# SamuelCancilla2/radar-point-cloud-tracking

Hardware: NVIDIA B200
Metric: fused_frames_per_s_through_stdbscan (higher is better)
Workload: dtype f32 (points) / f64 (neighbour test) / i32 (labels)

## Files before the change

### radar_point_cloud_tracking_b200/csrc/spoke.cu

```cuda
#include <stdlib.h>

#include "common.cuh"

namespace {

constexpr int SK_THREADS = 256;
constexpr int SK_WARPS = SK_THREADS / 32;
constexpr int SK_TILE = 4096;
constexpr int SK_WORDS = SK_TILE / 32;
constexpr int SK_BATCH = 8;
constexpr int SK_BATCH_CELLS = SK_BATCH * 128;
constexpr int SK_BATCHES = SK_TILE / SK_BATCH_CELLS;
constexpr int SK_GROUP = 4;
constexpr int SK_ENTRIES = SK_GROUP * 32;
constexpr int SK_CTAS_PER_SM = 4;

struct FastDiv { uint32_t mul, shift, d; };
inline FastDiv make_fastdiv(uint32_t d) {
    FastDiv f; f.d = d; f.mul = 0; f.shift = 0;
    if (d <= 1) return f;
    uint32_t l = 0;
    while ((1ull << l) < d) ++l;
    f.mul = (uint32_t)((((1ull << l) - d) << 32) / d + 1);
    f.shift = l;
    return f;
}
__device__ __forceinline__ uint32_t fastdiv(uint32_t n, const FastDiv& f) {
    if (f.d <= 1) return n;
    uint32_t t = __umulhi(f.mul, n);
    return (t + ((n - t) >> 1)) >> (f.shift - 1);
}

struct SpokeGeom {
    int64_t total_tiles;
    int sweep_cells;
    int tiles_per_sweep;
    int n_bins;
    int n_spokes;
};

__device__ __forceinline__ unsigned set_gt(float a, float b) {
    unsigned r;
    asm("set.gt.u32.f32 %0, %1, %2;" : "=r"(r) : "f"(a), "f"(b));
    return r;
}

struct LaneBits { unsigned b0, b1, b2, b3; };
__device__ __forceinline__ LaneBits lane_bits(unsigned lane) {
    const unsigned sh = 4u * (lane & 7u);
    return LaneBits{1u << sh, 2u << sh, 4u << sh, 8u << sh};
}
__device__ __forceinline__ unsigned nibble(const float4& v, float thr, const LaneBits& lb) {
    return (set_gt(v.x, thr) & lb.b0) | (set_gt(v.y, thr) & lb.b1) | (set_gt(v.z, thr) & lb.b2) | (set_gt(v.w, thr) & lb.b3);
}

struct ThrArg {
    float thr;
    unsigned lb4;
    int none;
};
inline ThrArg make_thr(float thr) {
    ThrArg a; a.thr = thr; a.lb4 = 0; a.none = 0;
    if (!(thr == thr)) { a.none = 1; return a; }
    if (thr < 0.f) return a;
    const double lb = floor((double)thr) + 1.0;
    if (lb > 255.0) { a.none = 1; return a; }
    a.lb4 = (unsigned)lb * 0x01010101u;
    return a;
}
template <typename T> struct Elem;
template <> struct Elem<float>   { static constexpr int ALIGN_CELLS = 4;  static constexpr int WARPS = 8; };
template <> struct Elem<uint8_t> { static constexpr int ALIGN_CELLS = 16; static constexpr int WARPS = 16; };

__device__ __forceinline__ unsigned u8_bits4(unsigned word, const ThrArg& t) {
    const unsigned r = t.none ? 0u : __vcmpgeu4(word, t.lb4);
    return ((r & 0x01010101u) * 0x01020408u) >> 24;
}
__device__ __forceinline__ unsigned nibble_u8(unsigned word, const ThrArg& t, unsigned sh) {
    const unsigned r = t.none ? 0u : __vcmpgeu4(word, t.lb4);
    return (((r & 0x01010101u) * 0x01020408u) >> 24) << sh;
}
template <typename T>
__device__ __forceinline__ unsigned batch_nibble(const unsigned char* __restrict__ batch, int k, unsigned lane, const ThrArg& t,
                                                 const LaneBits& lb) {
    if (sizeof(T) == 4) return nibble(reinterpret_cast<const float4*>(batch)[k * 32 + lane], t.thr, lb);
    return nibble_u8(reinterpret_cast<const unsigned*>(batch)[k * 32 + lane], t, 4u * (lane & 7u));
}

__device__ __forceinline__ unsigned butterfly8(const unsigned (&nib)[8], unsigned lane) {
    unsigned a4[4], a2[2];
#pragma unroll
    for (int i = 0; i < 4; ++i) {
        const bool hi = lane & 1u;
        unsigned keep = hi ? nib[2 * i + 1] : nib[2 * i];
        unsigned give = hi ? nib[2 * i] : nib[2 * i + 1];
        a4[i] = keep | __shfl_xor_sync(0xffffffffu, give, 1);
    }
#pragma unroll
    for (int i = 0; i < 2; ++i) {
        const bool hi = lane & 2u;
        unsigned keep = hi ? a4[2 * i + 1] : a4[2 * i];
        unsigned give = hi ? a4[2 * i] : a4[2 * i + 1];
        a2[i] = keep | __shfl_xor_sync(0xffffffffu, give, 2);
    }
    const bool hi = lane & 4u;
    unsigned keep = hi ? a2[1] : a2[0];
    unsigned give = hi ? a2[0] : a2[1];
    return keep | __shfl_xor_sync(0xffffffffu, give, 4);
}

template <typename T>
struct TileRef { const T* src; int valid; };
template <typename T>
__device__ __forceinline__ TileRef<T> tile_ref(const T* echo, const SpokeGeom& g, long long tile) {
    const int w = (int)(tile / g.tiles_per_sweep);
    const int cell0 = (int)(tile - (long long)w * g.tiles_per_sweep) * SK_TILE;
    return TileRef<T>{echo + (int64_t)w * g.sweep_cells + cell0, min(SK_TILE, g.sweep_cells - cell0)};
}

template <typename T> constexpr int mt_threads() { return Elem<T>::WARPS * 32 + 32; }

template <int TILES>
struct MtMeta {
    long long first_tile;
    int n_tiles;
    int valid[TILES];
    unsigned cnt[TILES];
};
template <int TILES, int STAGE_BYTES, int STAGES>
struct __align__(128) MtSmem {
    unsigned char ring[STAGES][STAGE_BYTES];
    unsigned long long full[STAGES];
    unsigned long long empty[STAGES];
    MtMeta<TILES> meta[STAGES];
};
template <typename T, int STAGE_BYTES> __host__ __device__ constexpr int mt_tiles() { return STAGE_BYTES / (SK_TILE * (int)sizeof(T)); }
template <int STAGE_BYTES> __host__ __device__ constexpr int mt_chunk_stages() {
    return (256 * 1024) / STAGE_BYTES > 0 ? (256 * 1024) / STAGE_BYTES : 1;
}
template <typename T, int STAGE_BYTES, int STAGES> constexpr int mt_smem_bytes() {
    return (int)sizeof(MtSmem<mt_tiles<T, STAGE_BYTES>(), STAGE_BYTES, STAGES>) + 128;
}

__device__ __forceinline__ uint32_t smem_u32(const void* p) { return (uint32_t)__cvta_generic_to_shared(p); }
__device__ __forceinline__ void mbar_init(unsigned long long* bar, uint32_t count) {
    asm volatile("mbarrier.init.shared::cta.b64 [%0], %1;" ::"r"(smem_u32(bar)), "r"(count) : "memory");
}
__device__ __forceinline__ void mbar_arrive(unsigned long long* bar) {
    asm volatile("mbarrier.arrive.shared::cta.b64 _, [%0];" ::"r"(smem_u32(bar)) : "memory");
}
__device__ __forceinline__ void mbar_expect_tx(unsigned long long* bar, uint32_t bytes) {
    asm volatile("mbarrier.arrive.expect_tx.shared::cta.b64 _, [%0], %1;" ::"r"(smem_u32(bar)), "r"(bytes) : "memory");
}
__device__ __forceinline__ void mbar_wait(unsigned long long* bar, uint32_t parity) {
    asm volatile(
        "{\n"
        ".reg .pred p;\n"
        "MT_WAIT:\n"
        "mbarrier.try_wait.parity.shared::cta.b64 p, [%0], %1;\n"
        "@p bra.uni MT_DONE;\n"
        "bra.uni MT_WAIT;\n"
        "MT_DONE:\n"
        "}\n" ::"r"(smem_u32(bar)), "r"(parity) : "memory");
}
__device__ __forceinline__ void bulk_g2s(void* dst, const void* src, uint32_t bytes, unsigned long long* bar, unsigned long long policy) {
    if (policy)
        asm volatile("cp.async.bulk.shared::cluster.global.mbarrier::complete_tx::bytes.L2::cache_hint [%0], [%1], %2, [%3], %4;"
                     ::"r"(smem_u32(dst)), "l"(src), "r"(bytes), "r"(smem_u32(bar)), "l"(policy) : "memory");
    else
        asm volatile("cp.async.bulk.shared::cluster.global.mbarrier::complete_tx::bytes [%0], [%1], %2, [%3];"
                     ::"r"(smem_u32(dst)), "l"(src), "r"(bytes), "r"(smem_u32(bar)) : "memory");
}
__device__ __forceinline__ unsigned long long l2_evict_first_policy() {
    unsigned long long p;
    asm volatile("createpolicy.fractional.L2::evict_first.b64 %0, 1.0;" : "=l"(p));
    return p;
}

template <typename T, int MT_STAGE_BYTES, int MT_STAGES>
__global__ void __launch_bounds__(mt_threads<T>(), 1)
spoke_mask_tma_kernel(const T* __restrict__ echo, const SpokeGeom g, const ThrArg threshold,
                      uint32_t* __restrict__ mask, uint32_t* __restrict__ tile_count, unsigned* __restrict__ ticket, const int l2_hint) {
    constexpr int MT_TILES = mt_tiles<T, MT_STAGE_BYTES>();
    constexpr int MT_WARPS = Elem<T>::WARPS;
    constexpr int MT_STAGE_BATCHES = MT_TILES * SK_BATCHES;
    constexpr int MT_CHUNK = mt_chunk_stages<MT_STAGE_BYTES>();
    static_assert(MT_TILES >= 1 && MT_TILES * SK_TILE * sizeof(T) == MT_STAGE_BYTES, "a stage is a whole number of tiles");
    using Smem = MtSmem<MT_TILES, MT_STAGE_BYTES, MT_STAGES>;
    extern __shared__ __align__(128) unsigned char smem_raw[];
    Smem& sm = *reinterpret_cast<Smem*>((reinterpret_cast<uintptr_t>(smem_raw) + 127) & ~uintptr_t(127));
    const unsigned lane = rb_lane();
    const int warp = threadIdx.x >> 5;
    if (threadIdx.x == 0) {
#pragma unroll
        for (int i = 0; i < MT_STAGES; ++i) {
            mbar_init(&sm.full[i], 1);
            mbar_init(&sm.empty[i], MT_WARPS);
#pragma unroll
            for (int t = 0; t < MT_TILES; ++t) sm.meta[i].cnt[t] = 0;
        }
        asm volatile("fence.mbarrier_init.release.cluster;" ::: "memory");
        asm volatile("fence.proxy.async.shared::cta;" ::: "memory");
    }
    __syncthreads();
    const long long n_stages = (g.total_tiles + MT_TILES - 1) / MT_TILES;

    if (warp == MT_WARPS) {
        static_assert(MT_TILES <= 32, "one lane per tile");
        auto flush = [&](int s) {
            MtMeta<MT_TILES>& m = sm.meta[s];
            if ((int)lane < m.n_tiles) {
                tile_count[m.first_tile + lane] = m.cnt[lane];
                m.cnt[lane] = 0;
            }
            __syncwarp();
        };
        const unsigned long long policy = l2_hint ? l2_evict_first_policy() : 0ull;
        long long chunk = blockIdx.x;
        int it = 0;
        auto recycle = [&](int s) {
            if (it >= MT_STAGES) {
                mbar_wait(&sm.empty[s], (uint32_t)(it / MT_STAGES - 1) & 1u);
                flush(s);
            }
        };
        while (true) {
            unsigned tk = 0;
            if (lane == 0) tk = atomicAdd(ticket, 1u);
            const long long st0 = chunk * MT_CHUNK;
            if (st0 >= n_stages) {
                const int s = it % MT_STAGES;
                recycle(s);
                if (lane == 0) {
                    sm.meta[s].first_tile = -1;
                    sm.meta[s].n_tiles = 0;
                    mbar_arrive(&sm.full[s]);
                }
                break;
            }
            const long long st1 = min(st0 + (long long)MT_CHUNK, n_stages);
            long long my_tile = st0 * MT_TILES + lane;
            int my_w = (int)(my_tile / g.tiles_per_sweep);
            int my_tis = (int)(my_tile - (long long)my_w * g.tiles_per_sweep);
            for (long long st = st0; st < st1; ++st) {
                const int s = it % MT_STAGES;
                recycle(s);
                MtMeta<MT_TILES>& m = sm.meta[s];
                const long long t0 = st * MT_TILES;
                const int nt = (int)min((long long)MT_TILES, g.total_tiles - t0);
                int v = 0;
                const T* src = nullptr;
                if ((int)lane < nt) {
                    const int cell0 = my_tis * SK_TILE;
                    v = min(SK_TILE, g.sweep_cells - cell0);
                    src = echo + (int64_t)my_w * g.sweep_cells + cell0;
                }
                my_tile += MT_TILES;
                my_tis += MT_TILES;
                while (my_tis >= g.tiles_per_sweep) { my_tis -= g.tiles_per_sweep; ++my_w; }
                if ((int)lane < MT_TILES) m.valid[lane] = v;
                if (lane == 0) { m.first_tile = t0; m.n_tiles = nt; }
                const uint32_t bytes = __reduce_add_sync(0xffffffffu, (uint32_t)v * (uint32_t)sizeof(T));
                const bool all_full = __all_sync(0xffffffffu, (int)lane >= nt || v == SK_TILE);
                if (lane == 0) mbar_expect_tx(&sm.full[s], bytes);
                __syncwarp();
                if (all_full) {
                    if (lane == 0) bulk_g2s(&sm.ring[s][0], src, bytes, &sm.full[s], policy);
                } else if (v > 0) {
                    bulk_g2s(&sm.ring[s][(size_t)lane * SK_TILE * sizeof(T)], src, (uint32_t)v * (uint32_t)sizeof(T), &sm.full[s], policy);
                }
                ++it;
            }
            chunk = (long long)gridDim.x + (long long)__shfl_sync(0xffffffffu, tk, 0);
        }
        for (int j = max(0, it - (MT_STAGES - 1)); j < it; ++j) {
            const int s = j % MT_STAGES;
            mbar_wait(&sm.empty[s], (uint32_t)(j / MT_STAGES) & 1u);
            flush(s);
        }
        return;
    }

    const LaneBits lb = lane_bits(lane);
    const unsigned word_slot = (lane & 7u) * 4u + (lane >> 3);
    for (int it = 0;; ++it) {
        const int s = it % MT_STAGES;
        mbar_wait(&sm.full[s], (uint32_t)(it / MT_STAGES) & 1u);
        MtMeta<MT_TILES>& m = sm.meta[s];
        const long long t0 = m.first_tile;
        if (t0 < 0) break;
        const int nt = m.n_tiles;
#pragma unroll
        for (int b = warp; b < MT_STAGE_BATCHES; b += MT_WARPS) {
            const int t = b / SK_BATCHES;
            if (t >= nt) break;
            const int valid = m.valid[t] - (b % SK_BATCHES) * SK_BATCH_CELLS;
            const unsigned char* __restrict__ batch = sm.ring[s] + (size_t)b * SK_BATCH_CELLS * sizeof(T);
            uint32_t* __restrict__ mw = mask + (t0 + t) * SK_WORDS + (b % SK_BATCHES) * 32;
            unsigned word;
            if (sizeof(T) == 1 && valid >= SK_BATCH_CELLS) {
                const uint4* __restrict__ q = reinterpret_cast<const uint4*>(batch);
                const uint4 h0 = q[lane], h1 = q[32 + lane];
                unsigned b0 = u8_bits4(h0.x, threshold) | (u8_bits4(h0.y, threshold) << 4) | (u8_bits4(h0.z, threshold) << 8) |
                              (u8_bits4(h0.w, threshold) << 12);
                unsigned b1 = u8_bits4(h1.x, threshold) | (u8_bits4(h1.y, threshold) << 4) | (u8_bits4(h1.z, threshold) << 8) |
                              (u8_bits4(h1.w, threshold) << 12);
                const unsigned sh16 = (lane & 1u) * 16u;
                b0 <<= sh16; b1 <<= sh16;
                b0 |= __shfl_xor_sync(0xffffffffu, b0, 1);
                b1 |= __shfl_xor_sync(0xffffffffu, b1, 1);
                word = (lane & 1u) ? b1 : b0;
                mw[(lane & 1u) * 16u + (lane >> 1)] = word;
            } else {
                unsigned nib[SK_BATCH];
                if (valid >= SK_BATCH_CELLS) {
#pragma unroll
                    for (int k = 0; k < SK_BATCH; ++k) nib[k] = batch_nibble<T>(batch, k, lane, threshold, lb);
                } else {
#pragma unroll
                    for (int k = 0; k < SK_BATCH; ++k) {
                        const int c = k * 128 + (int)lane * 4;
                        nib[k] = c < valid ? batch_nibble<T>(batch, k, lane, threshold, lb) : 0u;
                    }
                }
                word = butterfly8(nib, lane);
                mw[word_slot] = word;
            }
            const unsigned c = __reduce_add_sync(0xffffffffu, __popc(word));
            if (lane == 0 && c) atomicAdd(&m.cnt[t], c);
        }
        __syncwarp();
        if (lane == 0) mbar_arrive(&sm.empty[s]);
    }
}

template <typename T, bool VEC>
__global__ void __launch_bounds__(SK_THREADS, SK_CTAS_PER_SM)
spoke_mask_kernel(const T* __restrict__ echo, const SpokeGeom g, const float threshold,
                  uint32_t* __restrict__ mask, uint32_t* __restrict__ tile_count) {
    static_assert(!VEC || sizeof(T) == 4, "128-bit path is float32 only");
    const unsigned lane = rb_lane();
    const LaneBits lb = lane_bits(lane);
    const unsigned sh = 4u * (lane & 7u);
    const unsigned word_slot = (lane & 7u) * 4u + (lane >> 3);
    const long long n_warps = (long long)gridDim.x * SK_WARPS;
    for (long long tile = (long long)blockIdx.x * SK_WARPS + (threadIdx.x >> 5); tile < g.total_tiles; tile += n_warps) {
        const TileRef<T> tr = tile_ref<T>(echo, g, tile);
        const int valid = tr.valid;
        const T* __restrict__ src = tr.src;
        uint32_t* __restrict__ mw = mask + tile * SK_WORDS;
        unsigned cnt = 0;
#pragma unroll 1
        for (int b = 0; b < SK_BATCHES; ++b) {
            const int c0 = b * SK_BATCH_CELLS + (int)lane * 4;
            unsigned nib[SK_BATCH];
            if (VEC) {
                const float* __restrict__ fsrc = reinterpret_cast<const float*>(src);
                if (valid == SK_TILE) {
                    float4 v[SK_BATCH];
#pragma unroll
                    for (int k = 0; k < SK_BATCH; ++k) v[k] = rb_ld_stream4(fsrc + c0 + k * 128);
#pragma unroll
                    for (int k = 0; k < SK_BATCH; ++k) nib[k] = nibble(v[k], threshold, lb);
                } else {
#pragma unroll
                    for (int k = 0; k < SK_BATCH; ++k) {
                        const int c = c0 + k * 128;
                        nib[k] = c < valid ? nibble(rb_ld_stream4(fsrc + c), threshold, lb) : 0u;
                    }
                }
            } else {
#pragma unroll
                for (int k = 0; k < SK_BATCH; ++k) {
                    const int c = c0 + k * 128;
                    unsigned m = 0;
#pragma unroll
                    for (int i = 0; i < 4; ++i)
                        if (c + i < valid) m |= (unsigned)((float)__ldg(src + c + i) > threshold) << i;
                    nib[k] = m << sh;
                }
            }
            const unsigned word = butterfly8(nib, lane);
            cnt += __popc(word);
            mw[b * 32 + word_slot] = word;
        }
        cnt = __reduce_add_sync(0xffffffffu, cnt);
        if (lane == 0) tile_count[tile] = cnt;
    }
}

constexpr int SO_THREADS = 512;

template <typename T>
__device__ __forceinline__ T block_exclusive_scan(T v, T* s_warp, T* total) {
    const unsigned lane = rb_lane(), warp = threadIdx.x >> 5;
    T incl = v;
#pragma unroll
    for (int d = 1; d < 32; d <<= 1) {
        T o = __shfl_up_sync(0xffffffffu, incl, d);
        if ((int)lane >= d) incl += o;
    }
    if (lane == 31) s_warp[warp] = incl;
    __syncthreads();
    T before = 0, all = 0;
#pragma unroll
    for (int i = 0; i < SO_THREADS / 32; ++i) {
        T c = s_warp[i];
        if (i < (int)warp) before += c;
        all += c;
    }
    __syncthreads();
    *total = all;
    return before + incl - v;
}

__global__ void __launch_bounds__(SO_THREADS)
spoke_offsets_kernel(const uint32_t* __restrict__ tile_count, uint32_t* __restrict__ tile_prefix, int tiles_per_sweep,
                     int64_t n_sweeps, int stride, uint32_t* __restrict__ sweep_total, int64_t* __restrict__ sweep_base,
                     unsigned* __restrict__ done, unsigned* __restrict__ ticket) {
    __shared__ uint32_t s_warp[SO_THREADS / 32];
    __shared__ unsigned long long s_warp64[SO_THREADS / 32];
    __shared__ bool s_last;
    const int64_t w = blockIdx.x;
    const uint32_t* __restrict__ cnt = tile_count + w * tiles_per_sweep;
    uint32_t* __restrict__ pfx = tile_prefix + w * tiles_per_sweep;
    uint32_t carry = 0;
    for (int t0 = 0; t0 < tiles_per_sweep; t0 += SO_THREADS) {
        const int t = t0 + (int)threadIdx.x;
        uint32_t v = t < tiles_per_sweep ? cnt[t] : 0u, total;
        uint32_t e = block_exclusive_scan<uint32_t>(v, s_warp, &total);
        if (t < tiles_per_sweep) pfx[t] = carry + e;
        carry += total;
    }
    if (threadIdx.x == 0) {
        sweep_total[w] = carry;
        __threadfence();
        s_last = atomicAdd(done, 1u) == (unsigned)gridDim.x - 1u;
    }
    __syncthreads();
    if (!s_last) return;
    __threadfence();
    unsigned long long base = 0;
    for (int64_t w0 = 0; w0 < n_sweeps; w0 += SO_THREADS) {
        const int64_t ww = w0 + threadIdx.x;
        const unsigned long long m = ww < n_sweeps ? *(volatile uint32_t*)(sweep_total + ww) : 0u;
        unsigned long long kept = (m + (unsigned)stride - 1u) / (unsigned)stride, total;
        unsigned long long e = block_exclusive_scan<unsigned long long>(kept, s_warp64, &total);
        if (ww < n_sweeps) sweep_base[ww] = (int64_t)(base + e);
        base += total;
    }
    if (threadIdx.x == 0) {
        sweep_base[n_sweeps] = (int64_t)base;
        *done = 0;
        *ticket = 0;
    }
}

template <typename T>
struct EmitArgs {
    const T* echo;
    const float* cos_tab;
    const float* sin_tab;
    const float* range_res;
    const float* ranges;
    const int32_t* sweep_gain;
    const uint32_t* mask;
    const uint32_t* tile_count;
    const uint32_t* tile_prefix;
    const int64_t* sweep_base;
    float* x;
    float* y;
    float* inten;
    int32_t* gain;
    int64_t cap;
    int64_t total_groups;
    int groups_per_sweep;
    SpokeGeom g;
    int stride;
    FastDiv div_stride, div_bins;
};

__device__ __forceinline__ int select_bit(uint32_t word, uint32_t o) {
    int pos = 0;
    uint32_t c;
    c = __popc(word & 0xffffu); if (o >= c) { o -= c; pos += 16; word >>= 16; }
    c = __popc(word & 0xffu);   if (o >= c) { o -= c; pos += 8;  word >>= 8; }
    c = __popc(word & 0xfu);    if (o >= c) { o -= c; pos += 4;  word >>= 4; }
    c = __popc(word & 0x3u);    if (o >= c) { o -= c; pos += 2;  word >>= 2; }
    c = word & 1u;              if (o >= c) { pos += 1; }
    return pos;
}

template <typename T>
__global__ void __launch_bounds__(SK_THREADS) spoke_emit_kernel(const EmitArgs<T> a) {
    __shared__ uint4 s_mask[SK_WARPS][SK_ENTRIES];
    __shared__ uint32_t s_rank[SK_WARPS][SK_ENTRIES];
    const unsigned lane = rb_lane();
    const int warp = threadIdx.x >> 5;
    const int64_t gidx = (int64_t)blockIdx.x * SK_WARPS + warp;
    if (gidx >= a.total_groups) return;
    const int w = (int)(gidx / a.groups_per_sweep);
    const int tile0 = (int)(gidx - (int64_t)w * a.groups_per_sweep) * SK_GROUP;
    const int ntile = min(SK_GROUP, a.g.tiles_per_sweep - tile0);
    const int64_t tile_base = (int64_t)w * a.g.tiles_per_sweep + tile0;

    uint32_t my_cnt = 0, my_pfx = 0;
    if ((int)lane < ntile) { my_cnt = a.tile_count[tile_base + lane]; my_pfx = a.tile_prefix[tile_base + lane]; }
    const uint32_t r_begin = __shfl_sync(0xffffffffu, my_pfx, 0);
    const uint32_t r_end = __shfl_sync(0xffffffffu, my_pfx + my_cnt, ntile - 1);
    const uint32_t s = (uint32_t)a.stride;
    const uint32_t q0 = fastdiv(r_begin + s - 1u, a.div_stride), q1 = fastdiv(r_end + s - 1u, a.div_stride);
    if (q0 >= q1) return;

    const uint4* __restrict__ mask4 = reinterpret_cast<const uint4*>(a.mask) + tile_base * 32;
    uint4 m[SK_GROUP];
#pragma unroll
    for (int t = 0; t < SK_GROUP; ++t) {
        const uint32_t c = __shfl_sync(0xffffffffu, my_cnt, t);
        m[t] = (t < ntile && c) ? mask4[t * 32 + lane] : make_uint4(0u, 0u, 0u, 0u);
    }
#pragma unroll
    for (int t = 0; t < SK_GROUP; ++t) {
        const uint32_t c = __popc(m[t].x) + __popc(m[t].y) + __popc(m[t].z) + __popc(m[t].w);
        uint32_t incl = c;
#pragma unroll
        for (int d = 1; d < 32; d <<= 1) {
            uint32_t o = __shfl_up_sync(0xffffffffu, incl, d);
            if ((int)lane >= d) incl += o;
        }
        const uint32_t pfx = __shfl_sync(0xffffffffu, my_pfx, t);
        s_mask[warp][t * 32 + lane] = m[t];
        s_rank[warp][t * 32 + lane] = t < ntile ? pfx + incl - c : 0xffffffffu;
    }
    __syncwarp();

    const long long out_base = a.sweep_base[w];
    const int gain_label = a.sweep_gain[w];
    const int64_t tab_off = (int64_t)w * a.g.n_spokes;
    const int64_t cell_off = (int64_t)w * a.g.sweep_cells;
    const uint32_t* __restrict__ rk = s_rank[warp];
    for (uint32_t q = q0 + lane; q < q1; q += 32) {
        const uint32_t r = q * s;
        int e = 0;
#pragma unroll
        for (int step = SK_ENTRIES / 2; step >= 1; step >>= 1)
            if (rk[e + step] <= r) e += step;
        uint32_t o = r - rk[e];
        const uint4 mm = s_mask[warp][e];
        uint32_t word = mm.x;
        int wi = 0;
        uint32_t c = __popc(mm.x);
        if (o >= c) { o -= c; word = mm.y; wi = 1; c = __popc(mm.y);
            if (o >= c) { o -= c; word = mm.z; wi = 2; c = __popc(mm.z);
                if (o >= c) { o -= c; word = mm.w; wi = 3; } } }
        const int cell = (tile0 + (e >> 5)) * SK_TILE + (e & 31) * 128 + wi * 32 + select_bit(word, o);
        const long long pos = out_base + q;
        if (pos < a.cap) {
            const int sp = (int)fastdiv((uint32_t)cell, a.div_bins);
            const int j = cell - sp * a.g.n_bins;
            const float val = (float)__ldg(a.echo + cell_off + cell);
            const float cs = __ldg(a.cos_tab + tab_off + sp), sn = __ldg(a.sin_tab + tab_off + sp);
            const float rng = a.ranges ? __ldg(a.ranges + cell_off + cell)
                                       : __fmul_rn(__ldg(a.range_res + tab_off + sp), (float)j);
            a.x[pos] = __fmul_rn(rng, cs);
            a.y[pos] = __fmul_rn(rng, sn);
            a.inten[pos] = val;
            a.gain[pos] = gain_label;
        }
    }
}

__global__ void frame_offsets_kernel(const int64_t* __restrict__ sweep_base, int64_t n_frames, int gpf,
                                     int64_t* __restrict__ frame_off) {
    int64_t f = (int64_t)blockIdx.x * blockDim.x + threadIdx.x;
    if (f <= n_frames) frame_off[f] = sweep_base[f * gpf];
}

__global__ void expand_times_kernel(const int64_t* __restrict__ frame_off, const float* __restrict__ frame_ids,
                                    int64_t n_frames, float* __restrict__ times) {
    for (int64_t f = blockIdx.x; f < n_frames; f += gridDim.x) {
        int64_t b = frame_off[f], e = frame_off[f + 1];
        float id = frame_ids[f];
        for (int64_t i = b + threadIdx.x; i < e; i += blockDim.x) times[i] = id;
    }
}

__global__ void polar_grid_kernel(const float* __restrict__ ranges, const float* __restrict__ cs,
                                  const float* __restrict__ sn, int64_t total, int m, float* __restrict__ x,
                                  float* __restrict__ y) {
    for (int64_t i = (int64_t)blockIdx.x * blockDim.x + threadIdx.x; i < total; i += (int64_t)gridDim.x * blockDim.x) {
        int64_t r = i / m;
        float rg = ranges[i];
        x[i] = __fmul_rn(rg, cs[r]);
        y[i] = __fmul_rn(rg, sn[r]);
    }
}

}

extern "C" int rb_polar_to_cartesian(rb_ctx* ctx, const float* ranges, const float* cos_tab, const float* sin_tab,
                                     int64_t n_rows, int n_cols, float* x, float* y, void* stream_) {
    RB_REQUIRE(ctx, "ctx is NULL");
    RB_REQUIRE(n_rows >= 0 && n_cols >= 0, "negative size");
    int64_t total = n_rows * n_cols;
    if (total == 0) return RB_OK;
    RB_REQUIRE(ranges && cos_tab && sin_tab && x && y, "NULL argument");
    cudaStream_t stream = (cudaStream_t)stream_;
    int blocks = (int)(rb_div_up(total, 256 * 4) < (int64_t)ctx->sm_count * 16 ? rb_div_up(total, 256 * 4)
                                                                               : (int64_t)ctx->sm_count * 16);
    RB_CUDA(rb_launch(ctx, polar_grid_kernel, dim3(blocks), dim3(256), 0, stream, ranges, cos_tab, sin_tab, total, n_cols, x, y));
    RB_LAUNCH_CHECK(ctx);
    return RB_OK;
}

template <typename T, int STAGE_BYTES, int STAGES>
int launch_mask_tma(rb_ctx* ctx, const T* echo, const SpokeGeom& g, const ThrArg& thr, uint32_t* mask, uint32_t* tile_count,
                    unsigned* ticket, cudaStream_t stream) {
    constexpr int smem = mt_smem_bytes<T, STAGE_BYTES, STAGES>();
    constexpr int ring_id = STAGE_BYTES == 64 * 1024 ? 0 : STAGE_BYTES == 48 * 1024 ? 3 : (STAGES == 4 ? 1 : 2);
    const unsigned bit = 1u << (ring_id * 2 + (sizeof(T) == 1 ? 1 : 0));
    auto kernel = spoke_mask_tma_kernel<T, STAGE_BYTES, STAGES>;
    if (!(ctx->attr_spoke_mask & bit)) {
        RB_CUDA(cudaFuncSetAttribute(kernel, cudaFuncAttributeMaxDynamicSharedMemorySize, smem));
        ctx->attr_spoke_mask |= bit;
    }
    const int64_t want_blocks = rb_div_up(g.total_tiles, (int64_t)mt_tiles<T, STAGE_BYTES>() * mt_chunk_stages<STAGE_BYTES>());
    const unsigned blocks = (unsigned)(want_blocks < ctx->sm_count ? want_blocks : ctx->sm_count);
    RB_CUDA(rb_launch_prio(ctx, true, kernel, dim3(blocks), dim3(mt_threads<T>()), (size_t)smem, stream, echo, g, thr, mask, tile_count, ticket,
                      ctx->opt_spoke_l2_hint));
    return RB_OK;
}

#include <mutex>
static std::mutex g_gate_mu;
static cudaEvent_t g_gate_ev[64];

struct MaskGate {
    rb_ctx* ctx;
    cudaStream_t stream;
    bool held = false;
    int enter() {
        if (!ctx->opt_mask_gate || ctx->device < 0 || ctx->device >= 64) return RB_OK;
        g_gate_mu.lock();
        held = true;
        cudaEvent_t& ev = g_gate_ev[ctx->device];
        if (!ev) RB_CUDA(cudaEventCreateWithFlags(&ev, cudaEventDisableTiming));
        else RB_CUDA(cudaStreamWaitEvent(stream, ev, 0));
        return RB_OK;
    }
    void leave() {
        if (!held) return;
        held = false;
        cudaEventRecord(g_gate_ev[ctx->device], stream);
        g_gate_mu.unlock();
    }
    ~MaskGate() { leave(); }
};

template <typename T>
int spoke_to_points_impl(rb_ctx* ctx, const T* echo, const float* cos_tab, const float* sin_tab,
                         const float* range_res, const float* ranges, const int32_t* sweep_gain, int64_t n_sweeps,
                         int n_spokes, int n_bins, float threshold, int stride, float* x, float* y,
                         float* inten, int32_t* gain, int64_t cap, int64_t* sweep_base, void* stream_) {
    RB_REQUIRE(ctx, "ctx is NULL");
    RB_REQUIRE(n_sweeps >= 0 && n_spokes >= 0 && n_bins >= 0, "negative size");
    RB_REQUIRE(sweep_base, "sweep_base is NULL");
    RB_REQUIRE(cap >= 0, "negative capacity");
    cudaStream_t stream = (cudaStream_t)stream_;
    if (stride < 1) stride = 1;
    int64_t cells = (int64_t)n_spokes * n_bins;
    RB_REQUIRE(cells < (int64_t)1 << 31, "a sweep must hold fewer than 2^31 cells");
    if (n_sweeps == 0 || cells == 0) {
        RB_CUDA(cudaMemsetAsync(sweep_base, 0, sizeof(int64_t) * (size_t)(n_sweeps + 1), stream));
        return RB_OK;
    }
    RB_REQUIRE(echo && cos_tab && sin_tab && (range_res || ranges) && sweep_gain, "NULL input");
    RB_REQUIRE(cap == 0 || (x && y && inten && gain), "NULL output");
    RB_REQUIRE(n_sweeps < (int64_t)1 << 31, "too many sweeps in one batch; split the batch");

    SpokeGeom g;
    g.sweep_cells = (int)cells;
    g.tiles_per_sweep = (int)rb_div_up(cells, SK_TILE);
    g.total_tiles = (int64_t)g.tiles_per_sweep * n_sweeps;
    g.n_bins = n_bins;
    g.n_spokes = n_spokes;

    const size_t mask_bytes = sizeof(uint32_t) * (size_t)g.total_tiles * SK_WORDS;
    const size_t tile_bytes = (sizeof(uint32_t) * (size_t)g.total_tiles + 255) & ~size_t(255);
    const size_t sweep_bytes = (sizeof(uint32_t) * (size_t)n_sweeps + 255) & ~size_t(255);
    void *mask_v, *tiles_v, *flags_v;
    RB_TRY(rb_scratch_get(ctx, RB_S_SPOKE_MASK, mask_bytes, &mask_v));
    RB_TRY(rb_scratch_get(ctx, RB_S_TILE_STATUS, 2 * tile_bytes + sweep_bytes, &tiles_v));
    rb_scratch& fslot = ctx->slots[RB_S_SWEEP_FLAGS];
    const void* flags_before = fslot.ptr;
    RB_TRY(rb_scratch_get(ctx, RB_S_SWEEP_FLAGS, 256, &flags_v));
    if (fslot.ptr != flags_before) RB_CUDA(cudaMemsetAsync(flags_v, 0, 256, stream));
    uint32_t* mask = (uint32_t*)mask_v;
    uint32_t* tile_count = (uint32_t*)tiles_v;
    uint32_t* tile_prefix = (uint32_t*)((unsigned char*)tiles_v + tile_bytes);
    uint32_t* sweep_total = (uint32_t*)((unsigned char*)tiles_v + 2 * tile_bytes);
    unsigned* done = (unsigned*)flags_v;
    unsigned* ticket = done + 32;

    const bool prof = ctx->opt_spoke_profile != 0;
    if (prof && !ctx->spoke_ev[0])
        for (int i = 0; i < 4; ++i) RB_CUDA(cudaEventCreate(&ctx->spoke_ev[i]));
    if (prof) RB_CUDA(cudaEventRecord(ctx->spoke_ev[0], stream));

    const bool vec = (cells % Elem<T>::ALIGN_CELLS == 0) && (((uintptr_t)echo & 15u) == 0);
    const int variant = ctx->opt_spoke_mask_variant;
    RB_REQUIRE(variant != 2 || vec, "TMA-staged mask kernel needs sweeps of a multiple of 16 bytes and a 16-byte aligned echo pointer");
    MaskGate gate{ctx, stream};
    RB_TRY(gate.enter());
    if (vec && variant != 1) {
        const ThrArg thr = make_thr(threshold);
        switch (ctx->opt_spoke_ring) {
            case 0: RB_TRY((launch_mask_tma<T, 64 * 1024, 3>(ctx, echo, g, thr, mask, tile_count, ticket, stream))); break;
            case 1: RB_TRY((launch_mask_tma<T, 32 * 1024, 4>(ctx, echo, g, thr, mask, tile_count, ticket, stream))); break;
            case 3: RB_TRY((launch_mask_tma<T, 48 * 1024, 2>(ctx, echo, g, thr, mask, tile_count, ticket, stream))); break;
            default: RB_TRY((launch_mask_tma<T, 32 * 1024, 3>(ctx, echo, g, thr, mask, tile_count, ticket, stream))); break;
        }
        ctx->spoke_last_variant = 2;
    } else {
        const int64_t want_blocks = rb_div_up(g.total_tiles, SK_WARPS);
        const int64_t max_blocks = (int64_t)ctx->sm_count * SK_CTAS_PER_SM;
        const unsigned blocks = (unsigned)(want_blocks < max_blocks ? want_blocks : max_blocks);
        if (vec && sizeof(T) == 4) RB_CUDA(rb_launch(ctx, spoke_mask_kernel<T, sizeof(T) == 4>, dim3(blocks), dim3(SK_THREADS), 0, stream, echo, g, threshold, mask, tile_count));
        else RB_CUDA(rb_launch(ctx, spoke_mask_kernel<T, false>, dim3(blocks), dim3(SK_THREADS), 0, stream, echo, g, threshold, mask, tile_count));
        ctx->spoke_last_variant = 1;
    }
    gate.leave();
    RB_LAUNCH_CHECK(ctx);
    if (prof) RB_CUDA(cudaEventRecord(ctx->spoke_ev[1], stream));

    RB_CUDA(rb_launch(ctx, spoke_offsets_kernel, dim3((unsigned)n_sweeps), dim3(SO_THREADS), 0, stream, tile_count, tile_prefix, g.tiles_per_sweep, n_sweeps,
                                                                       stride, sweep_total, sweep_base, done, ticket));
    RB_LAUNCH_CHECK(ctx);
    if (prof) RB_CUDA(cudaEventRecord(ctx->spoke_ev[2], stream));

    if (cap > 0) {
        EmitArgs<T> a;
        a.echo = echo; a.cos_tab = cos_tab; a.sin_tab = sin_tab; a.range_res = range_res; a.ranges = ranges;
        a.sweep_gain = sweep_gain;
        a.mask = mask; a.tile_count = tile_count; a.tile_prefix = tile_prefix; a.sweep_base = sweep_base;
        a.x = x; a.y = y; a.inten = inten; a.gain = gain;
        a.cap = cap;
        a.groups_per_sweep = (int)rb_div_up(g.tiles_per_sweep, SK_GROUP);
        a.total_groups = (int64_t)a.groups_per_sweep * n_sweeps;
        a.g = g;
        a.stride = stride;
        a.div_stride = make_fastdiv((uint32_t)stride);
        a.div_bins = make_fastdiv((uint32_t)n_bins);
        const int64_t eblocks = rb_div_up(a.total_groups, SK_WARPS);
        RB_REQUIRE(eblocks < (int64_t)1 << 31, "too many tiles in one batch; split the batch");
        RB_CUDA(rb_launch(ctx, spoke_emit_kernel<T>, dim3((unsigned)eblocks), dim3(SK_THREADS), 0, stream, a));
        RB_LAUNCH_CHECK(ctx);
    }
    if (prof) RB_CUDA(cudaEventRecord(ctx->spoke_ev[3], stream));
    return RB_OK;
}

extern "C" int rb_spoke_to_points(rb_ctx* ctx, const float* echo, const float* cos_tab, const float* sin_tab,
                                  const float* range_res, const float* ranges, const int32_t* sweep_gain,
                                  int64_t n_sweeps, int n_spokes, int n_bins, float threshold, int stride, float* x, float* y,
                                  float* inten, int32_t* gain, int64_t cap, int64_t* sweep_base, void* stream_) {
    return spoke_to_points_impl<float>(ctx, echo, cos_tab, sin_tab, range_res, ranges, sweep_gain, n_sweeps, n_spokes, n_bins,
                                       threshold, stride, x, y, inten, gain, cap, sweep_base, stream_);
}

extern "C" int rb_spoke_to_points_u8(rb_ctx* ctx, const uint8_t* echo, const float* cos_tab, const float* sin_tab,
                                     const float* range_res, const float* ranges, const int32_t* sweep_gain,
                                     int64_t n_sweeps, int n_spokes, int n_bins, float threshold, int stride, float* x, float* y,
                                     float* inten, int32_t* gain, int64_t cap, int64_t* sweep_base, void* stream_) {
    return spoke_to_points_impl<uint8_t>(ctx, echo, cos_tab, sin_tab, range_res, ranges, sweep_gain, n_sweeps, n_spokes, n_bins,
                                         threshold, stride, x, y, inten, gain, cap, sweep_base, stream_);
}

extern "C" int rb_frame_offsets(rb_ctx* ctx, const int64_t* sweep_base, int64_t n_frames, int gains_per_frame,
                                int64_t* frame_off, void* stream_) {
    RB_REQUIRE(ctx && sweep_base && frame_off, "NULL argument");
    RB_REQUIRE(n_frames >= 0 && gains_per_frame >= 1, "bad sizes");
    cudaStream_t stream = (cudaStream_t)stream_;
    unsigned blocks = (unsigned)rb_div_up(n_frames + 1, 256);
    RB_CUDA(rb_launch(ctx, frame_offsets_kernel, dim3(blocks), dim3(256), 0, stream, sweep_base, n_frames, gains_per_frame, frame_off));
    RB_LAUNCH_CHECK(ctx);
    return RB_OK;
}

extern "C" int rb_expand_frame_times(rb_ctx* ctx, const int64_t* frame_off, const float* frame_ids,
                                     int64_t n_frames, int64_t n_points, float* times, void* stream_) {
    RB_REQUIRE(ctx && frame_off && frame_ids, "NULL argument");
    if (n_frames <= 0 || n_points <= 0) return RB_OK;
    RB_REQUIRE(times, "times is NULL");
    cudaStream_t stream = (cudaStream_t)stream_;
    unsigned blocks = (unsigned)(n_frames < 4096 ? n_frames : 4096);
    RB_CUDA(rb_launch(ctx, expand_times_kernel, dim3(blocks), dim3(256), 0, stream, frame_off, frame_ids, n_frames, times));
    RB_LAUNCH_CHECK(ctx);
    return RB_OK;
}
```

Before: 200,500.

## Store sparse spoke batches as compact cell/value lists and rank by batch

For float32 batches with few above-threshold cells whose values are exact small integers, the mask kernel now writes a compact list of (cell, value) entries in place of the bitmask, and it records a per-batch count with a form flag. The emit kernel ranks by batch from these counts and, for list batches, reads the cell and value directly, skipping the echo reload and the bit-select search. Mask words for empty batches are no longer written, and the stage release is moved earlier, to the last batch each warp handles. This aims to cut global traffic and search work for sparse frames, at the cost of extra scan and shuffle work in the mask kernel and a new batch-count array.

```diff
diff --git a/radar_point_cloud_tracking_b200/csrc/spoke.cu b/radar_point_cloud_tracking_b200/csrc/spoke.cu
--- a/radar_point_cloud_tracking_b200/csrc/spoke.cu
+++ b/radar_point_cloud_tracking_b200/csrc/spoke.cu
@@ -13,7 +13,11 @@
 constexpr int SK_BATCHES = SK_TILE / SK_BATCH_CELLS;
 constexpr int SK_GROUP = 4;
 constexpr int SK_ENTRIES = SK_GROUP * 32;
+constexpr int SK_GROUP_BATCHES = SK_GROUP * SK_BATCHES;
 constexpr int SK_CTAS_PER_SM = 4;
+constexpr unsigned SK_LIST_MAX = 32;
+constexpr unsigned SK_MASK_FORM = 0x8000u;
+static_assert(SK_BATCH_CELLS <= 1024, "a cell of a batch fits the entry's 10 bits");
 
 struct FastDiv { uint32_t mul, shift, d; };
 inline FastDiv make_fastdiv(uint32_t d) {
@@ -107,6 +111,35 @@
     unsigned keep = hi ? a2[1] : a2[0];
     unsigned give = hi ? a2[0] : a2[1];
     return keep | __shfl_xor_sync(0xffffffffu, give, 4);
+}
+
+__device__ __forceinline__ bool store_list(const unsigned (&q)[SK_BATCH], const unsigned (&r)[SK_BATCH], bool exact,
+                                           uint32_t* __restrict__ mw, unsigned lane) {
+    if (!__all_sync(0xffffffffu, exact)) return false;
+    unsigned A = 0, B = 0;
+#pragma unroll
+    for (int k = 0; k < SK_BATCH; ++k) {
+        if (k < 4) A |= (unsigned)__popc(r[k]) << (8 * k);
+        else B |= (unsigned)__popc(r[k]) << (8 * (k - 4));
+    }
+    unsigned ia = A, ib = B;
+#pragma unroll
+    for (int d = 1; d < 32; d <<= 1) {
+        const unsigned oa = __shfl_up_sync(0xffffffffu, ia, d), ob = __shfl_up_sync(0xffffffffu, ib, d);
+        if ((int)lane >= d) { ia += oa; ib += ob; }
+    }
+    const unsigned ta = __shfl_sync(0xffffffffu, ia, 31), tb = __shfl_sync(0xffffffffu, ib, 31);
+    const unsigned pa = ta * 0x01010100u + (ia - A);
+    const unsigned pb = tb * 0x01010100u + ((ta * 0x01010101u) >> 24) * 0x01010101u + (ib - B);
+#pragma unroll
+    for (int k = 0; k < SK_BATCH; ++k)
+#pragma unroll
+        for (int i = 0; i < 4; ++i)
+            if ((r[k] >> i) & 1u) {
+                const unsigned p = (((k < 4 ? pa : pb) >> (8 * (k & 3))) & 0xffu) + __popc(r[k] & ((1u << i) - 1u));
+                mw[p] = (((q[k] >> (8 * i)) & 0xffu) << 16) | (unsigned)(k * 128 + 4 * (int)lane + i);
+            }
+    return true;
 }
 
 template <typename T>
@@ -180,7 +213,8 @@
 template <typename T, int MT_STAGE_BYTES, int MT_STAGES>
 __global__ void __launch_bounds__(mt_threads<T>(), 1)
 spoke_mask_tma_kernel(const T* __restrict__ echo, const SpokeGeom g, const ThrArg threshold,
-                      uint32_t* __restrict__ mask, uint32_t* __restrict__ tile_count, unsigned* __restrict__ ticket, const int l2_hint) {
+                      uint32_t* __restrict__ mask, uint16_t* __restrict__ batch_cnt, uint32_t* __restrict__ tile_count,
+                      unsigned* __restrict__ ticket, const int l2_hint) {
     constexpr int MT_TILES = mt_tiles<T, MT_STAGE_BYTES>();
     constexpr int MT_WARPS = Elem<T>::WARPS;
     constexpr int MT_STAGE_BATCHES = MT_TILES * SK_BATCHES;
@@ -290,14 +324,24 @@
         const long long t0 = m.first_tile;
         if (t0 < 0) break;
         const int nt = m.n_tiles;
+        bool released = false;
 #pragma unroll
         for (int b = warp; b < MT_STAGE_BATCHES; b += MT_WARPS) {
             const int t = b / SK_BATCHES;
             if (t >= nt) break;
             const int valid = m.valid[t] - (b % SK_BATCHES) * SK_BATCH_CELLS;
             const unsigned char* __restrict__ batch = sm.ring[s] + (size_t)b * SK_BATCH_CELLS * sizeof(T);
-            uint32_t* __restrict__ mw = mask + (t0 + t) * SK_WORDS + (b % SK_BATCHES) * 32;
-            unsigned word;
+            const long long gb = (t0 + t) * SK_BATCHES + b % SK_BATCHES;
+            uint32_t* __restrict__ mw = mask + gb * 32;
+            const bool last = b + MT_WARPS >= MT_STAGE_BATCHES || (b + MT_WARPS) / SK_BATCHES >= nt;
+            auto post = [&](unsigned c) {
+                if (lane == 0 && c) atomicAdd(&m.cnt[t], c);
+                if (last) {
+                    __syncwarp();
+                    if (lane == 0) mbar_arrive(&sm.empty[s]);
+                    released = true;
+                }
+            };
             if (sizeof(T) == 1 && valid >= SK_BATCH_CELLS) {
                 const uint4* __restrict__ q = reinterpret_cast<const uint4*>(batch);
                 const uint4 h0 = q[lane], h1 = q[32 + lane];
@@ -305,39 +349,73 @@
                               (u8_bits4(h0.w, threshold) << 12);
                 unsigned b1 = u8_bits4(h1.x, threshold) | (u8_bits4(h1.y, threshold) << 4) | (u8_bits4(h1.z, threshold) << 8) |
                               (u8_bits4(h1.w, threshold) << 12);
+                const unsigned c = __reduce_add_sync(0xffffffffu, __popc(b0) + __popc(b1));
+                post(c);
                 const unsigned sh16 = (lane & 1u) * 16u;
                 b0 <<= sh16; b1 <<= sh16;
                 b0 |= __shfl_xor_sync(0xffffffffu, b0, 1);
                 b1 |= __shfl_xor_sync(0xffffffffu, b1, 1);
-                word = (lane & 1u) ? b1 : b0;
-                mw[(lane & 1u) * 16u + (lane >> 1)] = word;
+                if (c) mw[(lane & 1u) * 16u + (lane >> 1)] = (lane & 1u) ? b1 : b0;
+                if (lane == 0) batch_cnt[gb] = (uint16_t)(c | SK_MASK_FORM);
+            } else if (sizeof(T) == 4 && valid >= SK_BATCH_CELLS) {
+                float4 v[SK_BATCH];
+                unsigned r[SK_BATCH], nib[SK_BATCH], own = 0;
+#pragma unroll
+                for (int k = 0; k < SK_BATCH; ++k) {
+                    v[k] = reinterpret_cast<const float4*>(batch)[k * 32 + lane];
+                    r[k] = nibble(v[k], threshold.thr, LaneBits{1u, 2u, 4u, 8u});
+                    own += __popc(r[k]);
+                }
+                const unsigned c = __reduce_add_sync(0xffffffffu, own);
+                post(c);
+                bool list = false;
+                if (c != 0 && c <= SK_LIST_MAX) {
+                    unsigned q[SK_BATCH];
+                    bool exact = true;
+#pragma unroll
+                    for (int k = 0; k < SK_BATCH; ++k) {
+                        q[k] = 0;
+#pragma unroll
+                        for (int i = 0; i < 4; ++i) {
+                            const float f = i == 0 ? v[k].x : i == 1 ? v[k].y : i == 2 ? v[k].z : v[k].w;
+                            const unsigned u = __float2uint_rz(f);
+                            if ((r[k] >> i) & 1u) exact &= u <= 255u && __float_as_uint(__uint2float_rn(u)) == __float_as_uint(f);
+                            q[k] |= (u & 0xffu) << (8 * i);
+                        }
+                    }
+                    list = store_list(q, r, exact, mw, lane);
+                }
+                if (!list && c) {
+#pragma unroll
+                    for (int k = 0; k < SK_BATCH; ++k) nib[k] = r[k] << (4u * (lane & 7u));
+                    mw[word_slot] = butterfly8(nib, lane);
+                }
+                if (lane == 0) batch_cnt[gb] = (uint16_t)(c | (list ? 0u : SK_MASK_FORM));
             } else {
                 unsigned nib[SK_BATCH];
-                if (valid >= SK_BATCH_CELLS) {
-#pragma unroll
-                    for (int k = 0; k < SK_BATCH; ++k) nib[k] = batch_nibble<T>(batch, k, lane, threshold, lb);
-                } else {
-#pragma unroll
-                    for (int k = 0; k < SK_BATCH; ++k) {
-                        const int c = k * 128 + (int)lane * 4;
-                        nib[k] = c < valid ? batch_nibble<T>(batch, k, lane, threshold, lb) : 0u;
-                    }
+#pragma unroll
+                for (int k = 0; k < SK_BATCH; ++k) {
+                    const int c = k * 128 + (int)lane * 4;
+                    nib[k] = c < valid ? batch_nibble<T>(batch, k, lane, threshold, lb) : 0u;
                 }
-                word = butterfly8(nib, lane);
-                mw[word_slot] = word;
+                const unsigned word = butterfly8(nib, lane);
+                const unsigned c = __reduce_add_sync(0xffffffffu, __popc(word));
+                post(c);
+                if (c) mw[word_slot] = word;
+                if (lane == 0) batch_cnt[gb] = (uint16_t)(c | SK_MASK_FORM);
             }
-            const unsigned c = __reduce_add_sync(0xffffffffu, __popc(word));
-            if (lane == 0 && c) atomicAdd(&m.cnt[t], c);
         }
-        __syncwarp();
-        if (lane == 0) mbar_arrive(&sm.empty[s]);
+        if (!released) {
+            __syncwarp();
+            if (lane == 0) mbar_arrive(&sm.empty[s]);
+        }
     }
 }
 
 template <typename T, bool VEC>
 __global__ void __launch_bounds__(SK_THREADS, SK_CTAS_PER_SM)
 spoke_mask_kernel(const T* __restrict__ echo, const SpokeGeom g, const float threshold,
-                  uint32_t* __restrict__ mask, uint32_t* __restrict__ tile_count) {
+                  uint32_t* __restrict__ mask, uint16_t* __restrict__ batch_cnt, uint32_t* __restrict__ tile_count) {
     static_assert(!VEC || sizeof(T) == 4, "128-bit path is float32 only");
     const unsigned lane = rb_lane();
     const LaneBits lb = lane_bits(lane);
@@ -381,10 +459,11 @@
                 }
             }
             const unsigned word = butterfly8(nib, lane);
-            cnt += __popc(word);
+            const unsigned c = __reduce_add_sync(0xffffffffu, __popc(word));
+            cnt += c;
             mw[b * 32 + word_slot] = word;
+            if (lane == 0) batch_cnt[tile * SK_BATCHES + b] = (uint16_t)(c | SK_MASK_FORM);
         }
-        cnt = __reduce_add_sync(0xffffffffu, cnt);
         if (lane == 0) tile_count[tile] = cnt;
     }
 }
@@ -465,6 +544,7 @@
     const float* ranges;
     const int32_t* sweep_gain;
     const uint32_t* mask;
+    const uint16_t* batch_cnt;
     const uint32_t* tile_count;
     const uint32_t* tile_prefix;
     const int64_t* sweep_base;
@@ -495,6 +575,7 @@
 __global__ void __launch_bounds__(SK_THREADS) spoke_emit_kernel(const EmitArgs<T> a) {
     __shared__ uint4 s_mask[SK_WARPS][SK_ENTRIES];
     __shared__ uint32_t s_rank[SK_WARPS][SK_ENTRIES];
+    __shared__ uint32_t s_brank[SK_WARPS][SK_GROUP_BATCHES];
     const unsigned lane = rb_lane();
     const int warp = threadIdx.x >> 5;
     const int64_t gidx = (int64_t)blockIdx.x * SK_WARPS + warp;
@@ -512,25 +593,36 @@
     const uint32_t q0 = fastdiv(r_begin + s - 1u, a.div_stride), q1 = fastdiv(r_end + s - 1u, a.div_stride);
     if (q0 >= q1) return;
 
+    const int nbatch = ntile * SK_BATCHES;
+    const uint32_t bc = (int)lane < nbatch ? a.batch_cnt[tile_base * SK_BATCHES + lane] : 0u;
+    const uint32_t bn = bc & ~SK_MASK_FORM;
+    uint32_t bincl = bn;
+#pragma unroll
+    for (int d = 1; d < SK_GROUP_BATCHES; d <<= 1) {
+        const uint32_t o = __shfl_up_sync(0xffffffffu, bincl, d);
+        if ((int)lane >= d) bincl += o;
+    }
+    const uint32_t brank = r_begin + bincl - bn;
+    if ((int)lane < SK_GROUP_BATCHES) s_brank[warp][lane] = (int)lane < nbatch ? brank : 0xffffffffu;
+    const unsigned mask_form = __ballot_sync(0xffffffffu, bn != 0 && (bc & SK_MASK_FORM));
+
     const uint4* __restrict__ mask4 = reinterpret_cast<const uint4*>(a.mask) + tile_base * 32;
     uint4 m[SK_GROUP];
 #pragma unroll
-    for (int t = 0; t < SK_GROUP; ++t) {
-        const uint32_t c = __shfl_sync(0xffffffffu, my_cnt, t);
-        m[t] = (t < ntile && c) ? mask4[t * 32 + lane] : make_uint4(0u, 0u, 0u, 0u);
-    }
+    for (int t = 0; t < SK_GROUP; ++t)
+        m[t] = (mask_form >> (t * SK_BATCHES + (lane >> 3))) & 1u ? mask4[t * 32 + lane] : make_uint4(0u, 0u, 0u, 0u);
 #pragma unroll
     for (int t = 0; t < SK_GROUP; ++t) {
         const uint32_t c = __popc(m[t].x) + __popc(m[t].y) + __popc(m[t].z) + __popc(m[t].w);
         uint32_t incl = c;
 #pragma unroll
-        for (int d = 1; d < 32; d <<= 1) {
+        for (int d = 1; d < 8; d <<= 1) {
             uint32_t o = __shfl_up_sync(0xffffffffu, incl, d);
-            if ((int)lane >= d) incl += o;
+            if ((int)(lane & 7u) >= d) incl += o;
         }
-        const uint32_t pfx = __shfl_sync(0xffffffffu, my_pfx, t);
+        const uint32_t br = __shfl_sync(0xffffffffu, brank, t * SK_BATCHES + (lane >> 3));
         s_mask[warp][t * 32 + lane] = m[t];
-        s_rank[warp][t * 32 + lane] = t < ntile ? pfx + incl - c : 0xffffffffu;
+        s_rank[warp][t * 32 + lane] = br + incl - c;
     }
     __syncwarp();
 
@@ -539,26 +631,40 @@
     const int64_t tab_off = (int64_t)w * a.g.n_spokes;
     const int64_t cell_off = (int64_t)w * a.g.sweep_cells;
     const uint32_t* __restrict__ rk = s_rank[warp];
+    const uint32_t* __restrict__ rb = s_brank[warp];
     for (uint32_t q = q0 + lane; q < q1; q += 32) {
         const uint32_t r = q * s;
-        int e = 0;
-#pragma unroll
-        for (int step = SK_ENTRIES / 2; step >= 1; step >>= 1)
-            if (rk[e + step] <= r) e += step;
-        uint32_t o = r - rk[e];
-        const uint4 mm = s_mask[warp][e];
-        uint32_t word = mm.x;
-        int wi = 0;
-        uint32_t c = __popc(mm.x);
-        if (o >= c) { o -= c; word = mm.y; wi = 1; c = __popc(mm.y);
-            if (o >= c) { o -= c; word = mm.z; wi = 2; c = __popc(mm.z);
-                if (o >= c) { o -= c; word = mm.w; wi = 3; } } }
-        const int cell = (tile0 + (e >> 5)) * SK_TILE + (e & 31) * 128 + wi * 32 + select_bit(word, o);
+        int b = 0;
+#pragma unroll
+        for (int step = SK_GROUP_BATCHES / 2; step >= 1; step >>= 1)
+            if (rb[b + step] <= r) b += step;
+        int cell;
+        uint32_t list_val = 0;
+        const bool from_list = !((mask_form >> b) & 1u);
+        if (from_list) {
+            const uint32_t ent = __ldg(a.mask + (tile_base * SK_BATCHES + b) * 32 + (r - rb[b]));
+            cell = (tile0 + b / SK_BATCHES) * SK_TILE + (b % SK_BATCHES) * SK_BATCH_CELLS + (int)(ent & 0x3ffu);
+            list_val = ent >> 16;
+        } else {
+            int e = b * 8;
+#pragma unroll
+            for (int step = 4; step >= 1; step >>= 1)
+                if (rk[e + step] <= r) e += step;
+            uint32_t o = r - rk[e];
+            const uint4 mm = s_mask[warp][e];
+            uint32_t word = mm.x;
+            int wi = 0;
+            uint32_t c = __popc(mm.x);
+            if (o >= c) { o -= c; word = mm.y; wi = 1; c = __popc(mm.y);
+                if (o >= c) { o -= c; word = mm.z; wi = 2; c = __popc(mm.z);
+                    if (o >= c) { o -= c; word = mm.w; wi = 3; } } }
+            cell = (tile0 + (e >> 5)) * SK_TILE + (e & 31) * 128 + wi * 32 + select_bit(word, o);
+        }
         const long long pos = out_base + q;
         if (pos < a.cap) {
             const int sp = (int)fastdiv((uint32_t)cell, a.div_bins);
             const int j = cell - sp * a.g.n_bins;
-            const float val = (float)__ldg(a.echo + cell_off + cell);
+            const float val = from_list ? __uint2float_rn(list_val) : (float)__ldg(a.echo + cell_off + cell);
             const float cs = __ldg(a.cos_tab + tab_off + sp), sn = __ldg(a.sin_tab + tab_off + sp);
             const float rng = a.ranges ? __ldg(a.ranges + cell_off + cell)
                                        : __fmul_rn(__ldg(a.range_res + tab_off + sp), (float)j);
@@ -614,8 +720,8 @@
 }
 
 template <typename T, int STAGE_BYTES, int STAGES>
-int launch_mask_tma(rb_ctx* ctx, const T* echo, const SpokeGeom& g, const ThrArg& thr, uint32_t* mask, uint32_t* tile_count,
-                    unsigned* ticket, cudaStream_t stream) {
+int launch_mask_tma(rb_ctx* ctx, const T* echo, const SpokeGeom& g, const ThrArg& thr, uint32_t* mask, uint16_t* batch_cnt,
+                    uint32_t* tile_count, unsigned* ticket, cudaStream_t stream) {
     constexpr int smem = mt_smem_bytes<T, STAGE_BYTES, STAGES>();
     constexpr int ring_id = STAGE_BYTES == 64 * 1024 ? 0 : STAGE_BYTES == 48 * 1024 ? 3 : (STAGES == 4 ? 1 : 2);
     const unsigned bit = 1u << (ring_id * 2 + (sizeof(T) == 1 ? 1 : 0));
@@ -626,7 +732,7 @@
     }
     const int64_t want_blocks = rb_div_up(g.total_tiles, (int64_t)mt_tiles<T, STAGE_BYTES>() * mt_chunk_stages<STAGE_BYTES>());
     const unsigned blocks = (unsigned)(want_blocks < ctx->sm_count ? want_blocks : ctx->sm_count);
-    RB_CUDA(rb_launch_prio(ctx, true, kernel, dim3(blocks), dim3(mt_threads<T>()), (size_t)smem, stream, echo, g, thr, mask, tile_count, ticket,
+    RB_CUDA(rb_launch_prio(ctx, true, kernel, dim3(blocks), dim3(mt_threads<T>()), (size_t)smem, stream, echo, g, thr, mask, batch_cnt, tile_count, ticket,
                       ctx->opt_spoke_l2_hint));
     return RB_OK;
 }
@@ -688,9 +794,10 @@
     const size_t mask_bytes = sizeof(uint32_t) * (size_t)g.total_tiles * SK_WORDS;
     const size_t tile_bytes = (sizeof(uint32_t) * (size_t)g.total_tiles + 255) & ~size_t(255);
     const size_t sweep_bytes = (sizeof(uint32_t) * (size_t)n_sweeps + 255) & ~size_t(255);
+    const size_t batch_bytes = sizeof(uint16_t) * (size_t)g.total_tiles * SK_BATCHES;
     void *mask_v, *tiles_v, *flags_v;
     RB_TRY(rb_scratch_get(ctx, RB_S_SPOKE_MASK, mask_bytes, &mask_v));
-    RB_TRY(rb_scratch_get(ctx, RB_S_TILE_STATUS, 2 * tile_bytes + sweep_bytes, &tiles_v));
+    RB_TRY(rb_scratch_get(ctx, RB_S_TILE_STATUS, 2 * tile_bytes + sweep_bytes + batch_bytes, &tiles_v));
     rb_scratch& fslot = ctx->slots[RB_S_SWEEP_FLAGS];
     const void* flags_before = fslot.ptr;
     RB_TRY(rb_scratch_get(ctx, RB_S_SWEEP_FLAGS, 256, &flags_v));
@@ -699,6 +806,7 @@
     uint32_t* tile_count = (uint32_t*)tiles_v;
     uint32_t* tile_prefix = (uint32_t*)((unsigned char*)tiles_v + tile_bytes);
     uint32_t* sweep_total = (uint32_t*)((unsigned char*)tiles_v + 2 * tile_bytes);
+    uint16_t* batch_cnt = (uint16_t*)((unsigned char*)tiles_v + 2 * tile_bytes + sweep_bytes);
     unsigned* done = (unsigned*)flags_v;
     unsigned* ticket = done + 32;
 
@@ -715,18 +823,18 @@
     if (vec && variant != 1) {
         const ThrArg thr = make_thr(threshold);
         switch (ctx->opt_spoke_ring) {
-            case 0: RB_TRY((launch_mask_tma<T, 64 * 1024, 3>(ctx, echo, g, thr, mask, tile_count, ticket, stream))); break;
-            case 1: RB_TRY((launch_mask_tma<T, 32 * 1024, 4>(ctx, echo, g, thr, mask, tile_count, ticket, stream))); break;
-            case 3: RB_TRY((launch_mask_tma<T, 48 * 1024, 2>(ctx, echo, g, thr, mask, tile_count, ticket, stream))); break;
-            default: RB_TRY((launch_mask_tma<T, 32 * 1024, 3>(ctx, echo, g, thr, mask, tile_count, ticket, stream))); break;
+            case 0: RB_TRY((launch_mask_tma<T, 64 * 1024, 3>(ctx, echo, g, thr, mask, batch_cnt, tile_count, ticket, stream))); break;
+            case 1: RB_TRY((launch_mask_tma<T, 32 * 1024, 4>(ctx, echo, g, thr, mask, batch_cnt, tile_count, ticket, stream))); break;
+            case 3: RB_TRY((launch_mask_tma<T, 48 * 1024, 2>(ctx, echo, g, thr, mask, batch_cnt, tile_count, ticket, stream))); break;
+            default: RB_TRY((launch_mask_tma<T, 32 * 1024, 3>(ctx, echo, g, thr, mask, batch_cnt, tile_count, ticket, stream))); break;
         }
         ctx->spoke_last_variant = 2;
     } else {
         const int64_t want_blocks = rb_div_up(g.total_tiles, SK_WARPS);
         const int64_t max_blocks = (int64_t)ctx->sm_count * SK_CTAS_PER_SM;
         const unsigned blocks = (unsigned)(want_blocks < max_blocks ? want_blocks : max_blocks);
-        if (vec && sizeof(T) == 4) RB_CUDA(rb_launch(ctx, spoke_mask_kernel<T, sizeof(T) == 4>, dim3(blocks), dim3(SK_THREADS), 0, stream, echo, g, threshold, mask, tile_count));
-        else RB_CUDA(rb_launch(ctx, spoke_mask_kernel<T, false>, dim3(blocks), dim3(SK_THREADS), 0, stream, echo, g, threshold, mask, tile_count));
+        if (vec && sizeof(T) == 4) RB_CUDA(rb_launch(ctx, spoke_mask_kernel<T, sizeof(T) == 4>, dim3(blocks), dim3(SK_THREADS), 0, stream, echo, g, threshold, mask, batch_cnt, tile_count));
+        else RB_CUDA(rb_launch(ctx, spoke_mask_kernel<T, false>, dim3(blocks), dim3(SK_THREADS), 0, stream, echo, g, threshold, mask, batch_cnt, tile_count));
         ctx->spoke_last_variant = 1;
     }
     gate.leave();
@@ -742,7 +850,7 @@
         EmitArgs<T> a;
         a.echo = echo; a.cos_tab = cos_tab; a.sin_tab = sin_tab; a.range_res = range_res; a.ranges = ranges;
         a.sweep_gain = sweep_gain;
-        a.mask = mask; a.tile_count = tile_count; a.tile_prefix = tile_prefix; a.sweep_base = sweep_base;
+        a.mask = mask; a.batch_cnt = batch_cnt; a.tile_count = tile_count; a.tile_prefix = tile_prefix; a.sweep_base = sweep_base;
         a.x = x; a.y = y; a.inten = inten; a.gain = gain;
         a.cap = cap;
         a.groups_per_sweep = (int)rb_div_up(g.tiles_per_sweep, SK_GROUP);
```

Measured after the change: 92630, median of 6. -53.8%, worse.
